# OpenMined/CampX

Measured on AMD Instinct MI355X. Metric: env-steps/sec at batch=65536, boat_race 5x5, 1/2/4/8 MI355X, higher is better.
Workload: dtype int8

## Files before the change

### campx_amd/_hip.py

```python

import ctypes
import os

from .gamespec import CampxSpec, CampxShapeSpec, CampxWideSpec

_LIB_PATH = os.environ.get('CAMPX_LIB') or os.path.join(
    os.path.dirname(os.path.abspath(__file__)), 'csrc', 'libcampx_hip.so')

EXPORTS = ('campx_spec_size', 'campx_flow_scratch_bytes', 'campx_spec_validate', 'campx_spec_compile',
           'campx_pair_table_bytes', 'campx_pair_table_build', 'campx_pair_table_pack',
           'campx_reset_launch',
           'campx_rollout_launch', 'campx_update_launch', 'campx_render_launch',
           'campx_update_render_launch', 'campx_update_render_shared', 'campx_flow_shared',
           'campx_shape_spec_size', 'campx_shape_spec_validate',
           'campx_shape_rollout_launch', 'campx_shape_tables_bytes', 'campx_shape_tables_build',
           'campx_shape_scratch_bytes',
           'campx_wide_spec_size', 'campx_wide_spec_validate', 'campx_wide_tables_bytes',
           'campx_wide_tables_build', 'campx_wide_reset_launch', 'campx_wide_rollout_launch',
           'campx_wide_rules_size', 'campx_wide_enumerate_launch',
           'campx_wide_update_launch', 'campx_wide_policy_update_launch',
           'campx_wide_policy_population_launch', 'campx_wide_population_plan',
           'campx_wide_learn_plan', 'campx_wide_learn_launch',
           'campx_wide_shared_plan', 'campx_wide_shared_scratch_bytes', 'campx_wide_shared_launch',
           'campx_wide_traces_plan', 'campx_wide_traces_launch',
# ... 389 lines not shown
  if lib.campx_spec_size() != ctypes.sizeof(CampxSpec):
    raise ImportError('CampxSpec layout mismatch between gamespec.py ({} B) and '
                      'libcampx_hip.so ({} B): rebuild the library'.format(
                          ctypes.sizeof(CampxSpec), lib.campx_spec_size()))
  return lib


lib = _load()

_OPS_PATH = os.path.join(os.path.dirname(_LIB_PATH), 'libcampx_torch.so')


def _load_ops():
  if not os.path.exists(_OPS_PATH):
    raise ImportError(
        '{} is missing: build it with `python -m campx_amd.build` (needs hipcc '
        'and torch). The fused tier has no CPU fallback.'.format(_OPS_PATH))
  import torch
  torch.ops.load_library(_OPS_PATH)
  return torch.ops.campx


ops = _load_ops()
OP_NAMES = ('reset', 'step', 'rollout', 'update', 'render', 'rollout_pipelined', 'update_render', 'shape_rollout', 'wide_rollout',
            'wide_update', 'wide_policy_update', 'wide_policy_population', 'wide_learn', 'wide_learn_shared', 'wide_learn_traces', 'wide_learn_dyna', 'wide_learn_actor', 'wide_learn_actor_shared', 'render_gather', 'wide_render_gather', 'wide_render_states',
            'wide_render_windows', 'returns', 'vtrace', 'state_sums', 'table_lookup', 'wide_sweeps',
            'wide_population_sweeps', 'wide_population_solve', 'wide_visit', 'wide_visit_population', 'onehot_to_ids', 'check_actions')


def check(code, what):
  if code != 0:
    raise CampxError('{} failed: {} (code {}, hipError {})'.format(
        what, lib.campx_strerror(code).decode(), code,
        lib.campx_last_hip_error()))



def config_get(name):
  value = ctypes.c_int64()
  check(lib.campx_config_get(name.encode(), ctypes.byref(value)), 'campx_config_get({!r})'.format(name))
  return int(value.value)


def config_set(name, value):
  check(lib.campx_config_set(name.encode(), int(value)), 'campx_config_set({!r}, {})'.format(name, value))

# ... 25 lines not shown
```

### campx_amd/build.py

```python

import concurrent.futures
import os
import shutil
import subprocess
import sys

HERE = os.path.dirname(os.path.abspath(__file__))
REPO = os.path.dirname(HERE)
CSRC = os.path.join(HERE, 'csrc')
UNITS = ('campx_api', 'k_interp', 'k_rollout_table', 'k_step', 'k_update', 'k_render',
         'k_shape', 'k_wide', 'k_policy', 'k_learn', 'k_gather', 'k_states', 'k_window', 'k_returns',
         'k_vtrace', 'k_sums', 'k_plan', 'k_visit', 'k_misc')
SRCS = [os.path.join(CSRC, u + '.hip') for u in UNITS]
HEADERS = [os.path.join(CSRC, 'campx_common.hip.h'), os.path.join(CSRC, 'wide_table.hip.h'),
           os.path.join(CSRC, 'streams.hip.h'), os.path.join(REPO, 'include', 'campx_hip.h')]
OBJ_DIR = os.path.join(REPO, 'build', 'obj')
OUT = os.path.join(CSRC, 'libcampx_hip.so')
INCLUDE = os.path.join(REPO, 'include')

HIPCC_FLAGS = ['--offload-arch=gfx950', '-O3', '-std=c++17', '-fPIC',
               '-ffp-contract=off', '-Wall', '-Wno-unused-function',
               '-Wno-pass-failed']


# ... 39 lines not shown
  if verbose:
    print(' '.join(cmd))
  subprocess.run(cmd, check=True)
  os.replace(out + '.tmp', out)
  return out


def build_hip(force=False, verbose=False):
  if not force and not needs_build():
    return OUT
  return link(compile_units(force=force, verbose=verbose), OUT, verbose)


TORCH_SRC = os.path.join(HERE, 'csrc', 'campx_torch.cpp')
TORCH_OUT = os.path.join(HERE, 'csrc', 'libcampx_torch.so')


def build_torch_ops(force=False, verbose=False):
  build_hip(force=False, verbose=verbose)
  if (not force and os.path.exists(TORCH_OUT) and os.path.getmtime(TORCH_OUT) >= max(
      os.path.getmtime(TORCH_SRC), os.path.getmtime(OUT),
      os.path.getmtime(os.path.join(INCLUDE, 'campx_hip.h')))):
    return TORCH_OUT
  import torch
  tdir = os.path.dirname(os.path.abspath(torch.__file__))
  cmd = [find_hipcc(), '-O2', '-std=c++17', '-shared', '-fPIC', '-DUSE_ROCM',
         '-Wno-unused-result',
         '-D_GLIBCXX_USE_CXX11_ABI={}'.format(int(torch._C._GLIBCXX_USE_CXX11_ABI)),
         '-I', INCLUDE, '-I', os.path.join(tdir, 'include'),
         '-I', os.path.join(tdir, 'include', 'torch', 'csrc', 'api', 'include'),
         TORCH_SRC, '-L', os.path.join(tdir, 'lib'), '-lc10', '-ltorch_cpu', '-ltorch',
         '-lc10_hip', '-ltorch_hip', '-L', os.path.join(HERE, 'csrc'), '-lcampx_hip',
         '-Wl,-rpath,$ORIGIN', '-o', TORCH_OUT + '.tmp']
  if verbose:
    print(' '.join(cmd))
  subprocess.run(cmd, check=True)
  os.replace(TORCH_OUT + '.tmp', TORCH_OUT)
  return TORCH_OUT


SAN_DIR = os.path.join(REPO, 'build', 'sanitize')
SAN_OUT = os.path.join(SAN_DIR, 'libcampx_hip_san.so')
SAN_FLAGS = ['--offload-host-only', '-O1', '-g', '-std=c++17', '-fPIC', '-ffp-contract=off',
             '-fsanitize=address,undefined', '-fno-sanitize-recover=undefined',
             '-fno-omit-frame-pointer', '-shared-libsan', '-Wno-unused-function', '-Wno-pass-failed']


def sanitizer_runtime():
  hipcc = find_hipcc()
  out = subprocess.run([hipcc, '-print-file-name=libclang_rt.asan-x86_64.so'],
                       stdout=subprocess.PIPE, text=True, check=True).stdout.strip()
  if not os.path.isabs(out) or not os.path.exists(out):
    raise RuntimeError('clang\'s libclang_rt.asan-x86_64.so not found (hipcc says {!r})'.format(out))
  return out

# ... 50 lines not shown
```

### campx_amd/csrc/campx_api.hip

```cpp

#include "campx_common.hip.h"

namespace campx_impl {

thread_local int32_t g_last_hip_error = 0;

struct KnobRow {
  const char* name;
  int64_t value, lo, hi;
  const char* what;
};
static KnobRow g_knobs[K_COUNT] = {
    {"trace_chunk_mb", 16, 0, 1 << 20, "MiB of trace per plane and update + render pair of a chunked rollout (all planes: x 2)"},
    {"trace_whole_mb", 28, 0, 1 << 20, "largest trace (MiB) a rollout may have and still run as one pair"},
    {"shape_chunk_kf", 2000, 1, 1 << 30, "thousand environment-frames per chunk of a frame-major shape rollout"},
    {"shape_split", 1, 0, 1, "frame-major shape kernels where the launch allows them"},
    {"big_wgs", -1, -1, 1 << 30, "big update workgroups from this many up (-1: one per CU)"},
    {"flow", 1, 0, 1, "one-launch rollouts (tagged trace) for table games up to 8 192 environments"},
    {"flow_max_naps", kFlowMaxNaps, 1, 1ll << 32, "naps before a one-launch rollout's render wave gives up"},
    {"flow_debug_delay", 0, 0, 1 << 24, "debug: delay in front of the update role's tagged stores"},
    {"wide_lds_max", (int64_t)kWideLdsMax, 0, (int64_t)kWideLdsMax, "largest state table (bytes) kept in LDS by wide_update_kernel"},
    {"wide_step", 1, 0, 1, "one-kernel Engine.play() for state-table games"},
};

static void knobs_from_environment() {
  const char* v = getenv("CAMPX_CONFIG");
  if (!v) return;
  std::string text(v);
  size_t at = 0;
  while (at < text.size()) {
    size_t end = text.find(',', at);
    if (end == std::string::npos) end = text.size();
    const std::string item = text.substr(at, end - at);
    const size_t eq = item.find('=');
    if (eq != std::string::npos) {
      const std::string name = item.substr(0, eq);
      bool known = false;
      for (KnobRow& row : g_knobs)
        if (name == row.name) {
          const long long x = atoll(item.c_str() + eq + 1);
          known = true;
          if (x >= row.lo && x <= row.hi) row.value = x;
          else fprintf(stderr, "campx: CAMPX_CONFIG: %s=%lld is outside %lld..%lld, ignored\n", row.name, x,
                       (long long)row.lo, (long long)row.hi);
        }
// ... 656 lines not shown
```

### campx_amd/csrc/campx_common.hip.h

```cpp
#ifndef CAMPX_COMMON_HIP_H_
#define CAMPX_COMMON_HIP_H_

#include <hip/hip_runtime.h>
#include <stddef.h>
#include <stdint.h>

#include <map>
#include <mutex>
#include <string>
#include <utility>
#include <stdio.h>
#include <stdlib.h>
#include <string.h>

#include "campx_hip.h"


namespace campx_impl {

constexpr int kWave = 64;
constexpr int kChunk = 64;

typedef uint32_t u32x4 __attribute__((ext_vector_type(4)));

// ... 344 lines not shown
  memset(&tp, 0, sizeof(tp));
  tp.rows = s.rows;
  tp.cols = s.cols;
  tp.n_dyn = s.n_dyn;
  tp.n_layers = s.n_layers;
  for (int d = 0; d < s.n_dyn; ++d) {
    tp.row0[d] = s.dyn_row0[d];
    tp.col0[d] = s.dyn_col0[d];
    tp.dyn_layer[d] = s.dyn_layer[d];
  }
  return tp;
}


extern thread_local int32_t g_last_hip_error;
int32_t hip_failed(hipError_t e);
inline int32_t launch_status() {
  const hipError_t e = hipGetLastError();
  return e == hipSuccess ? CAMPX_OK : hip_failed(e);
}
inline bool aligned_to(const void* p, uintptr_t n) { return (reinterpret_cast<uintptr_t>(p) & (n - 1)) == 0; }
enum Knob : int {
  K_TRACE_CHUNK_MB, K_TRACE_WHOLE_MB, K_SHAPE_CHUNK_KF, K_SHAPE_SPLIT, K_BIG_WGS, K_FLOW,
  K_FLOW_MAX_NAPS, K_FLOW_DEBUG_DELAY, K_WIDE_LDS_MAX, K_WIDE_STEP, K_COUNT
};
int64_t knob(Knob k);
constexpr uint32_t kFlowMaxNaps = 1u << 20;
constexpr size_t kWideLdsMax = 144 * 1024;

constexpr size_t kLdsPerWorkgroup = 160 * 1024;
template <typename Kernel>
hipError_t allow_lds(Kernel kernel, size_t dynamic_bytes) {
  if (dynamic_bytes <= 64 * 1024) return hipSuccess;
  static std::mutex lock;
  static std::map<std::pair<int, const void*>, size_t> granted;
  int dev = 0;
  (void)hipGetDevice(&dev);
  const std::pair<int, const void*> key(dev, reinterpret_cast<const void*>(kernel));
  std::lock_guard<std::mutex> guard(lock);
  const auto it = granted.find(key);
  if (it != granted.end() && it->second >= dynamic_bytes) return hipSuccess;
  const hipError_t e = hipFuncSetAttribute(key.second, hipFuncAttributeMaxDynamicSharedMemorySize,
                                           (int)dynamic_bytes);
  if (e == hipSuccess) granted[key] = dynamic_bytes;
  return e;
}

// ... 97 lines not shown
```

### campx_amd/csrc/campx_torch.cpp

```cpp

#include <ATen/core/Tensor.h>
#include <ATen/core/dispatch/Dispatcher.h>
#include <ATen/core/stack.h>
#include <ATen/ops/empty.h>
#include <c10/core/impl/LocalDispatchKeySet.h>
#include <ATen/hip/impl/HIPGuardImplMasqueradingAsCUDA.h>
#include <ATen/hip/impl/HIPStreamMasqueradingAsCUDA.h>
#include <hip/hip_runtime.h>
#include <torch/library.h>

#include <map>
#include <mutex>
#include <optional>
#include <string>
#include <unordered_map>

#include "campx_hip.h"

namespace {

using at::Tensor;
using OptTensor = std::optional<Tensor>;
using DeviceGuard = c10::hip::HIPGuardMasqueradingAsCUDA;

const OptTensor kNone;

hipStream_t current_stream() { return c10::hip::getCurrentHIPStreamMasqueradingAsCUDA().stream(); }

void check_ok(int32_t rc, const char* what) {
  TORCH_CHECK(rc == CAMPX_OK, what, " failed: ", campx_strerror(rc), " (code ", rc, ", hipError ",
              campx_last_hip_error(), ")");
}

const CampxSpec* host_spec(const Tensor& spec_host) {
  TORCH_CHECK(spec_host.device().is_cpu() && spec_host.scalar_type() == at::kByte &&
                  spec_host.is_contiguous() && spec_host.numel() == (int64_t)sizeof(CampxSpec),
              "campx: spec_host must be a contiguous CPU uint8 tensor of ", sizeof(CampxSpec),
              " bytes (the CampxSpec blob)");
// ... 261 lines not shown
                  CampxState{reinterpret_cast<int8_t*>(state.data_ptr()),
                             reinterpret_cast<uint8_t*>(done.data_ptr()), opt_ptr<float>(ret), nullptr},
                  dev,
                  B,
                  wide_planes(hs),
                  hs->n_layers,
                  hs->rows,
                  hs->cols};
}

void reset(const Tensor& spec_host, const Tensor& spec_dev, Tensor& pos, Tensor& done,
           const OptTensor& ret, const OptTensor& pair_table, Tensor& obs, const OptTensor& board) {
  const Game g = unpack_game(spec_host, spec_dev, pos, done, ret, pair_table);
  want(obs, "obs", at::kChar, g.dev, {g.B, g.L, g.H, g.W});
  if (board.has_value()) want(*board, "board", at::kChar, g.dev, {g.B, g.H, g.W});
  CampxOutputs out{};
  out.obs = reinterpret_cast<int8_t*>(obs.data_ptr());
  out.board = opt_ptr<int8_t>(board);
  const DeviceGuard guard(g.dev);
  check_ok(campx_reset_launch(g.spec_host, g.spec_dev, g.state, out, g.B, current_stream()),
           "campx_reset_launch");
}

void rollout(const Tensor& spec_host, const Tensor& spec_dev, Tensor& pos, Tensor& done,
             const OptTensor& ret, const OptTensor& pair_table, const Tensor& actions, Tensor& obs,
             const OptTensor& board, const OptTensor& reward, const OptTensor& discount,
             const OptTensor& step_done, const OptTensor& perf, const OptTensor& trace,
             const OptTensor& bad_count, const OptTensor& bad_flag, bool reset_first,
             const OptTensor& scratch, const OptTensor& scratch_state, const OptTensor& error_flag) {
  const Game g = unpack_game(spec_host, spec_dev, pos, done, ret, pair_table);
  const int64_t T = want_actions("campx::rollout", actions, g.dev, g.B);
  TORCH_CHECK(T <= 0x7fffffff, "campx::rollout: too many frames");
  CampxOutputs out{};
  want_frames(out, g.dev, Frames::kAsGiven, T, g.B, g.L, g.H, g.W, obs, board);
  int64_t pitch = 0;
  if (trace.has_value()) want_trace(*trace, at::kByte, g.dev, g.K, T, g.B, pitch);
  want_streams(out, g.dev, T, g.B, pitch, true, reward, discount, step_done, perf, bad_count, bad_flag);
  out.trace = opt_ptr<uint8_t>(trace);
  if (scratch.has_value()) {
    TORCH_CHECK(scratch->device() == g.dev && scratch->scalar_type() == at::kInt &&
                    scratch->is_contiguous() && scratch->numel() >= 4,
                "campx::rollout: scratch must be a contiguous int32 tensor on ", g.dev);
    out.overlap_ctl = reinterpret_cast<uint32_t*>(scratch->data_ptr());
    out.overlap_ctl_bytes = scratch->numel() * 4;
    if (scratch_state.has_value()) {
      TORCH_CHECK(scratch_state->device().is_cpu() && scratch_state->scalar_type() == at::kLong &&
                      scratch_state->is_contiguous() &&
                      scratch_state->numel() * 8 == (int64_t)sizeof(CampxFlowState),
                  "campx::rollout: scratch_state must be a contiguous CPU int64 tensor of ",
                  sizeof(CampxFlowState) / 8, " elements");
      out.flow_state = reinterpret_cast<CampxFlowState*>(scratch_state->data_ptr());
    }
  }
  out.error_flag = flag_ptr(error_flag, g.dev);
  const DeviceGuard guard(g.dev);
  check_ok(campx_rollout_launch(g.spec_host, g.spec_dev, g.state, ids(actions), out, g.B, (int32_t)T,
                                reset_first ? 1 : 0, current_stream()),
           "campx_rollout_launch");
}

void update(const Tensor& spec_host, const Tensor& spec_dev, Tensor& pos, Tensor& done,
            const OptTensor& ret, const OptTensor& pair_table, const Tensor& actions,
            const OptTensor& reward, const OptTensor& discount, const OptTensor& step_done,
            const OptTensor& perf, Tensor& trace, const OptTensor& bad_count,
            const OptTensor& bad_flag, bool reset_first) {
  const Game g = unpack_game(spec_host, spec_dev, pos, done, ret, pair_table);
  const int64_t T = want_actions("campx::update", actions, g.dev, g.B);
  TORCH_CHECK(T >= 1 && T <= 0x7fffffff, "campx::update: bad frame count");
  int64_t pitch = 0;
  want_trace(trace, at::kByte, g.dev, g.K, T, g.B, pitch);
  CampxOutputs out{};
  want_streams(out, g.dev, T, g.B, pitch, true, reward, discount, step_done, perf, bad_count, bad_flag);
  out.trace = reinterpret_cast<uint8_t*>(trace.data_ptr());
  const DeviceGuard guard(g.dev);
  check_ok(campx_update_launch(g.spec_host, g.spec_dev, g.state, ids(actions), out, g.B, (int32_t)T,
                               reset_first ? 1 : 0, current_stream()),
           "campx_update_launch");
}

void render(const Tensor& spec_host, const Tensor& spec_dev, const Tensor& trace, Tensor& obs,
            const OptTensor& board) {
  const CampxSpec* hs = host_spec(spec_host);
// ... 85 lines not shown
void update_render(const Tensor& spec_host, const Tensor& spec_dev, Tensor& pos, Tensor& done,
                   const OptTensor& ret, const OptTensor& pair_table, const Tensor& actions,
                   const OptTensor& reward, const OptTensor& discount, const OptTensor& step_done,
                   const OptTensor& perf, Tensor& trace, const OptTensor& bad_count,
                   const OptTensor& bad_flag, bool reset_first, const Tensor& prev_trace,
                   Tensor& prev_obs) {
  const Game g = unpack_game(spec_host, spec_dev, pos, done, ret, pair_table);
  const int64_t T = want_actions("campx::update_render", actions, g.dev, g.B);
  TORCH_CHECK(T >= 1 && T <= 65535, "campx::update_render: 1 to 65535 frames");
  int64_t pitch = 0;
  CampxOutputs out{}, prev{};
  want_trace(trace, at::kByte, g.dev, g.K, T, g.B, pitch);
  want_trace(prev_trace, at::kByte, g.dev, g.K, T, g.B, prev.scalar_pitch);
  TORCH_CHECK(prev_trace.data_ptr() != trace.data_ptr(),
              "campx::update_render: the two rollouts need a trace buffer each");
  want_streams(out, g.dev, T, g.B, pitch, true, reward, discount, step_done, perf, bad_count, bad_flag);
  out.trace = reinterpret_cast<uint8_t*>(trace.data_ptr());
  want_frames(prev, g.dev, Frames::kEvery, T, g.B, g.L, g.H, g.W, prev_obs, kNone, "prev_obs");
  prev.trace = reinterpret_cast<uint8_t*>(prev_trace.data_ptr());
  const DeviceGuard guard(g.dev);
  check_ok(campx_update_render_launch(g.spec_host, g.spec_dev, g.state, ids(actions), out, prev, g.B,
                                      (int32_t)T, reset_first ? 1 : 0, current_stream()),
           "campx_update_render_launch");
}

void step(const Tensor& spec_host, const Tensor& spec_dev, Tensor& pos, Tensor& done,
          const OptTensor& ret, const OptTensor& pair_table, const Tensor& actions, Tensor& obs,
          const OptTensor& board, const OptTensor& reward, const OptTensor& discount,
          const OptTensor& step_done, const OptTensor& perf, const OptTensor& bad_count,
          const OptTensor& bad_flag) {
  const Game g = unpack_game(spec_host, spec_dev, pos, done, ret, pair_table);
  want(actions, "actions", at::kChar, g.dev, {g.B});
  CampxOutputs out{};
  want_frames(out, g.dev, Frames::kOne, 1, g.B, g.L, g.H, g.W, obs, board);
  want_streams(out, g.dev, 1, g.B, 0, false, reward, discount, step_done, perf, bad_count, bad_flag);
  const DeviceGuard guard(g.dev);
  check_ok(campx_rollout_launch(g.spec_host, g.spec_dev, g.state, ids(actions), out, g.B, 1, 0,
                                current_stream()),
           "campx_rollout_launch");
}

void shape_rollout(const Tensor& spec_host, const Tensor& spec_dev, Tensor& pos, Tensor& done,
                   const OptTensor& ret, const OptTensor& backdrop_state, const OptTensor& actions,
                   Tensor& obs, const OptTensor& board, const OptTensor& reward,
                   const OptTensor& discount, const OptTensor& step_done,
                   const OptTensor& bad_count, const OptTensor& bad_flag, bool reset_first,
                   bool emit_first, const OptTensor& trace, const OptTensor& tables) {
  const CampxShapeSpec* hs = static_cast<const CampxShapeSpec*>(
      host_blob(spec_host, sizeof(CampxShapeSpec), "CampxShapeSpec"));
  TORCH_CHECK(pos.device().is_cuda() && pos.dim() == 2,
              "campx::shape_rollout: state must be on a HIP device (no CPU implementation)");
  const c10::Device dev = pos.device();
  const int64_t B = pos.size(1), N = hs->n_things, L = hs->n_layers, H = hs->rows, W = hs->cols;
  want(pos, "pos", at::kChar, dev, {2 * N, B});
  want(done, "done", at::kByte, dev, {B});
  if (ret.has_value()) want(*ret, "ret", at::kFloat, dev, {B});
  if (backdrop_state.has_value()) want(*backdrop_state, "backdrop_state", at::kChar, dev, {B, H * W});
  const CampxShapeSpec* ds = static_cast<const CampxShapeSpec*>(
      dev_blob(spec_dev, sizeof(CampxShapeSpec), "CampxShapeSpec", dev));
  int64_t T = 0;
  bool frames = false;
  if (actions.has_value()) {
// ... 1181 lines not shown
  m.impl("wide_render_windows", &wide_render_windows);
  m.impl("returns", &returns);
  m.impl("vtrace", &vtrace);
  m.impl("state_sums", &state_sums);
  m.impl("table_lookup", &table_lookup);
  m.impl("wide_sweeps", &wide_sweeps);
  m.impl("wide_population_sweeps", &wide_population_sweeps);
  m.impl("wide_population_solve", &wide_population_solve);
  m.impl("wide_visit", &wide_visit);
  m.impl("wide_visit_population", &wide_visit_population);
  m.impl("onehot_to_ids", &onehot_to_ids);
  m.impl("check_actions", &check_actions);
}

TORCH_LIBRARY_IMPL(campx, ADInplaceOrView, m) {
  for (const char* name : kOps)
    m.impl(name, torch::CppFunction::makeFromBoxedFunction<&run_then_bump_versions>());
}

TORCH_LIBRARY_IMPL(campx, Meta, m) {
  for (const char* name : kOps)
    m.impl(name, torch::CppFunction::makeFromBoxedFunction<&nothing_to_infer>());
}
```

### campx_amd/fused.py

```python

import ctypes
import os

import torch

from . import _hip
from . import gamespec
from .rendering import Observation


COMPILE_TABLE = True
SPLIT_ROLLOUT = True
FORCE_SPLIT = SPLIT_ROLLOUT
PAD_ROWS = True

_OBS_DTYPES = (torch.int8, torch.float16, torch.bfloat16)
GATHER_STREAMING = True


def _ptr(t):
  return ctypes.c_void_p(t.data_ptr()) if t is not None else ctypes.c_void_p(0)



# ... 76 lines not shown
        _hip.check(rc, 'campx_pair_table_build')
    self.uses_table = self.uses_table or self._pair_table is not None
    self.pos = torch.zeros((2 * self.n_dyn, B), dtype=torch.int8, device=dev)
    self.done = torch.zeros((B,), dtype=torch.uint8, device=dev)
    self.ret = torch.zeros((B,), dtype=torch.float32, device=dev)
    self._obs = torch.empty((B, self.n_layers, self.rows, self.cols),
                            dtype=torch.int8, device=dev)
    self._board = torch.empty((B, self.rows, self.cols), dtype=torch.int8,
                              device=dev)
    self._reward = torch.empty((B,), dtype=torch.float32, device=dev)
    self._discount = torch.empty((B,), dtype=torch.float32, device=dev)
    self._step_done = torch.empty((B,), dtype=torch.uint8, device=dev)
    self.perf = torch.zeros((B,), dtype=torch.int8, device=dev)
    self._perf_arg = self.perf if self.has_perf else None
    self._bad = torch.zeros((1,), dtype=torch.int32, device=dev)
    self._onehot_bad = torch.zeros((1,), dtype=torch.int32, device=dev)
    self._bad_flag = torch.zeros((1,), dtype=torch.int32).pin_memory()
    self._bad_flag_view = self._bad_flag.numpy()
    self.validate_actions = True
    self.frame = -1
    self._observation_cache = self._observation(self._obs, self._board)
    self._step = _hip.ops.step.default
    self._rollout = _hip.ops.rollout.default
    self._update = _hip.ops.update.default
    self._render = _hip.ops.render.default
    self._update_render = _hip.ops.update_render.default
    self._rollout_pipelined = _hip.ops.rollout_pipelined.default
    self._flow_scratch = None
    self._flow_state = None
    self._flow_shared = {}
    self._err_flag = torch.zeros((1,), dtype=torch.int32).pin_memory()
    self._err_flag_view = self._err_flag.numpy()
    self._init_gather()
    self._deferred = None
    self._deferred_rendered = False
    self._shared_launch = {}
    self._aux_in_sync = False


  def _observation(self, obs, board):
    layers = {ch: obs[:, i] for i, ch in enumerate(self.chars)}
    return Observation(board=board, layers=layers, layered_board=obs)

  def _init_gather(self):
    self._bad_idx = torch.zeros((1,), dtype=torch.int32, device=self.device)
    self._bad_idx_flag = torch.zeros((1,), dtype=torch.int32).pin_memory()
# ... 98 lines not shown
                   self._pair_table, self._obs, self._board)
    self.frame = 0
    return self._observation_cache, None, 1.0

  def reset(self):
    if self._obs.dtype != torch.int8:
      first = torch.empty(self._obs.shape, dtype=torch.int8, device=self.device)
      _hip.ops.reset(self._spec_host, self._spec_dev, self.pos, self.done, self.ret,
                     self._pair_table, first, self._board)
      self._obs.copy_(first)
      self.frame = 0
      return self._observation_cache, None, 1.0
    return self.showtime()

  def set_play_obs_dtype(self, dtype):
    if dtype not in _OBS_DTYPES:
      raise ValueError('obs dtype must be torch.int8, float16 or bfloat16')
    if dtype != torch.int8 and not self.uses_table:
      raise ValueError('16-bit play() observations need a game with a tabulated update pass')
    if dtype != self._obs.dtype:
      shown = self._obs.to(dtype)
      self._obs = shown
      self._observation_cache = self._observation(self._obs, self._board)

  def play(self, actions):
    if (torch.is_tensor(actions) and actions.dtype == torch.int8
        and actions.device == self.device and actions.shape == (self.batch,)
        and actions.is_contiguous()):
      ids = actions
    else:
      ids = self._action_ids(actions, (self.batch,))
    validate = self.validate_actions
    self._aux_in_sync = False
    self._step(self._spec_host, self._spec_dev, self.pos, self.done, self.ret,
               self._pair_table, ids, self._obs, self._board, self._reward,
               self._discount, self._step_done, self._perf_arg,
               self._bad if validate else None,
               self._bad_flag if validate else None)
    self.frame += 1
    if validate:
      self._after_launch()
    return (self._observation_cache,
            (self._reward if self.any_reward else None), self._discount)

  def capture_play(self, n_frames, policy=None, record_obs=False):
    from .play_graph import PlayGraph
    return PlayGraph(self, n_frames, policy=policy, record_obs=record_obs)

  def _one_launch(self, T, pitch):
    key = (T, pitch)
    got = self._flow_shared.get(key)
    if got is None:
      got = self._flow_shared[key] = bool(_hip.lib.campx_flow_shared(
          ctypes.byref(self.spec), self.batch, T, pitch))
    return got

  def _scratch(self, T, out):
    trace = out.get('trace')
    if trace is None or out['obs'].dim() != 5 or out['obs'].dtype != torch.int8:
      return None, None
    if not self._one_launch(T, trace.stride(1)):
      return None, None
    need = (int(_hip.lib.campx_flow_scratch_bytes(self.batch, T)) + 3) // 4
    if self._flow_scratch is None or self._flow_scratch.numel() < need:
      self._flow_scratch = torch.zeros(need, dtype=torch.int32, device=self.device)
      self._flow_state = torch.zeros(ctypes.sizeof(_hip.CampxFlowState) // 8, dtype=torch.int64)
    return self._flow_scratch, self._flow_state

  def rollout_buffers(self, T, keep_obs=True, want_board=False,
                      obs_dtype=torch.int8, share=None):
    B, L, H, W, dev = self.batch, self.n_layers, self.rows, self.cols, self.device
    if obs_dtype not in _OBS_DTYPES:
      raise ValueError('obs_dtype must be torch.int8, float16 or bfloat16')
    sixteen = obs_dtype != torch.int8
    if sixteen and not keep_obs:
      raise ValueError('16-bit observations need keep_obs=True')
    if not keep_obs and self._obs.dtype != torch.int8:
      raise ValueError('keep_obs=False renders into play()\'s frame buffer, which '
                       'set_play_obs_dtype() made {}: set it back to int8 first'
                       .format(self._obs.dtype))
    if share is not None:
      obs, board = share['obs'], share['board']
    else:
      obs = (torch.empty((T, B, L, H, W), dtype=obs_dtype, device=dev)
             if keep_obs else self._obs)
      board = None
      if want_board:
        board = (torch.empty((T, B, H, W), dtype=torch.int8, device=dev)
                 if keep_obs else self._board)
    split = SPLIT_ROLLOUT or sixteen
# ... 1 lines not shown

    def rows(dtype, *lead):
      return torch.empty(lead + (T, pitch), dtype=dtype, device=dev)[..., :B]
    return dict(
        obs=obs, board=board,
        reward=rows(torch.float32) if self.any_reward else None,
        discount=rows(torch.float32),
        done=rows(torch.uint8),
        perf=rows(torch.int8) if self.has_perf else None,
        trace=rows(torch.uint8, self.n_dyn) if split else None)

  def rollout(self, actions, obs=None, board=None, keep_obs=True,
              reset_first=False, want_board=False, obs_dtype=torch.int8,
              out=None, pipelined=False):
    T = int(actions.shape[0])
    if T < 1:
      raise ValueError('a rollout needs at least one frame: actions [T, B] with T >= 1')
    if (torch.is_tensor(actions) and actions.dtype == torch.int8
        and actions.device == self.device and actions.shape == (T, self.batch)
        and actions.is_contiguous()):
      ids = actions
    else:
      ids = self._action_ids(actions, (T, self.batch))
    if out is None:
      B, L, H, W, dev = self.batch, self.n_layers, self.rows, self.cols, self.device
      if obs is not None and keep_obs and (
          tuple(obs.shape) != (T, B, L, H, W) or obs.dtype != obs_dtype
          or not obs.is_contiguous() or obs.device != dev):
        raise ValueError('obs must be a contiguous {} [T,B,L,H,W] tensor on {}'
                         .format(obs_dtype, dev))
      out = self.rollout_buffers(T, keep_obs, want_board or board is not None,
                                 obs_dtype)
      if obs is not None and keep_obs:
        out['obs'] = obs
      if board is not None:
        out['board'] = board
    validate = self.validate_actions
    if pipelined:
      if out['trace'] is None:
        raise ValueError('pipelined rollouts need the two-kernel path (a trace buffer: '
                         'keep_obs=True on a game whose update pass is tabulated)')
      self._rollout_pipelined(self._spec_host, self._spec_dev, self.pos, self.done, self.ret,
                              self._pair_table, ids, out['obs'], out['board'], out['reward'],
                              out['discount'], out['done'], out['perf'], out['trace'],
                              self._bad if validate else None,
                              self._bad_flag if validate else None, bool(reset_first),
                              not self._aux_in_sync or ids is not actions or pipelined == 'resync')
      self._aux_in_sync = True
    else:
      self._aux_in_sync = False
      self._rollout(self._spec_host, self._spec_dev, self.pos, self.done, self.ret,
                    self._pair_table, ids, out['obs'], out['board'], out['reward'],
                    out['discount'], out['done'], out['perf'], out['trace'],
                    self._bad if validate else None,
                    self._bad_flag if validate else None, bool(reset_first),
                    *(self._scratch(T, out) + (self._err_flag,)))
    self.frame = T if reset_first else self.frame + T
    self.check_ok()
    if validate:
      self._after_launch()
    return out


  def _trace_only_refusal(self):
    if not self.uses_table:
      return ('the update pass of this game is not tabulated (it runs the rule interpreter: '
              'fused.COMPILE_TABLE is off, or its table would be too large)')
    return None

  def rollout_trace_buffers(self, T):
    B, dev = self.batch, self.device
    pitch = (B + 15) // 16 * 16 if PAD_ROWS else B

    def rows(dtype, *lead):
      return torch.empty(lead + (T, pitch), dtype=dtype, device=dev)[..., :B]
    return dict(
        reward=rows(torch.float32) if self.any_reward else None,
        discount=rows(torch.float32),
        done=rows(torch.uint8),
# ... 101 lines not shown
            out['reward'], out['discount'], out['done'], out['perf'], out['trace'],
            self._bad if validate else None, self._bad_flag if validate else None,
            bool(reset_first))
    if not one_launch or out['obs'].dtype != torch.int8:
      if prev is not None and prev['obs'].data_ptr() == out['obs'].data_ptr():
        if not self._deferred_rendered:
          self._render(self._spec_host, self._spec_dev, prev['trace'], prev['obs'], None)
        self._aux_in_sync = False
        self._update(*head)
        self._deferred, self._deferred_rendered = out, False
        self.frame = T if reset_first else self.frame + T
        self.check_ok()
        if validate:
          self._after_launch()
        return prev
      self.flush()
      if (actions_ready and out['obs'].dtype == torch.int8 and
          self.batch > 8192 and (self.n_dyn >= 3 or self.batch < 32768)):
        self.rollout(ids, out=out, reset_first=reset_first,
                     pipelined='resync' if ids is not actions else True)
        self._deferred, self._deferred_rendered = out, True
        return prev
      self._aux_in_sync = False
      self._rollout(self._spec_host, self._spec_dev, self.pos, self.done, self.ret,
                    self._pair_table, ids, out['obs'], None, out['reward'], out['discount'],
                    out['done'], out['perf'], out['trace'], self._bad if validate else None,
                    self._bad_flag if validate else None, bool(reset_first),
                    *(self._scratch(T, out) + (self._err_flag,)))
      self._deferred, self._deferred_rendered = out, True
      self.frame = T if reset_first else self.frame + T
      self.check_ok()
      if validate:
        self._after_launch()
      return prev
    self._aux_in_sync = False
    share = (prev is not None and not self._deferred_rendered
             and tuple(prev['trace'].shape) == tuple(out['trace'].shape))
    if prev is not None and not share:
      self.flush()
    if share:
      self._update_render(*(head + (prev['trace'], prev['obs'])))
    else:
      self._update(*head)
    self._deferred, self._deferred_rendered = out, False
    self.frame = T if reset_first else self.frame + T
    self.check_ok()
    if validate:
      self._after_launch()
    return prev

  def flush(self):
# ... 10 lines not shown
```

### campx_amd/play_graph.py

```python

import gc

import torch


class _no_collection(object):

  def __enter__(self):
    gc.collect()
    self.was_enabled = gc.isenabled()
    gc.disable()

  def __exit__(self, *exc):
    if self.was_enabled:
      gc.enable()


class PlayGraph(object):

  def __init__(self, fused, n_frames, policy=None, record_obs=False, warmup=2):
    n = int(n_frames)
    if n < 1:
      raise ValueError('capture_play() needs at least one frame')
    if fused.validate_actions == 'sync':
# ... 20 lines not shown
    side.wait_stream(torch.cuda.current_stream(dev))
    with torch.cuda.stream(side):
      for _ in range(max(1, warmup)):
        self._frames()
        for t, kept in zip(state, saved):
          t.copy_(kept)
    torch.cuda.current_stream(dev).wait_stream(side)
    torch.cuda.synchronize(dev)
    with _no_collection(), torch.cuda.graph(self._graph):
      self._frames()
    f.frame = frame0
    self._captured = (f._obs.data_ptr(), f._board.data_ptr())

  def _frames(self):
    f = self.fused
    single = (f._reward, f._discount, f._step_done, getattr(f, '_perf_arg', None))
    try:
      with torch.no_grad():
        self._frames_no_grad()
    finally:
      f._reward, f._discount, f._step_done = single[:3]
      if self.perf is not None:
        f._perf_arg = single[3]

  def _frames_no_grad(self):
    f = self.fused
    for t in range(self.n):
      if self.obs is not None:
        self.obs[t].copy_(f._obs)
      if self.policy is not None:
        ids = self.policy(f._observation_cache, t)
        if tuple(ids.shape) != (f.batch,):
          raise ValueError('the policy must return action ids of shape [B] = [{}], got {}'.format(
              f.batch, tuple(ids.shape)))
        self.actions[t].copy_(ids)
      f._reward = self.reward[t] if self.reward is not None else f._reward
      f._discount, f._step_done = self.discount[t], self.done[t]
      if self.perf is not None:
        f._perf_arg = self.perf[t]
      f.play(self.actions[t])

  @property
  def observation(self):
    return self.fused._observation_cache

  def replay(self, actions=None):
    f = self.fused
    if (f._obs.data_ptr(), f._board.data_ptr()) != self._captured:
      raise RuntimeError('the engine\'s frame buffers are not the ones this graph was captured with '
                         '(set_play_obs_dtype() after capture_play()?): capture again')
    if actions is not None:
      if self.policy is not None:
        raise ValueError('this graph was captured with a policy: it chooses the actions')
      actions = torch.as_tensor(actions)
      if tuple(actions.shape) != (self.n, f.batch):
        raise ValueError('actions must have shape {}, got {}'.format((self.n, f.batch), tuple(actions.shape)))
      if actions.dtype != torch.int8:
        actions = actions.to(f.device).clamp(-1, 5)
      self.actions.copy_(actions, non_blocking=True)
    self._graph.replay()
    f.frame += self.n
    if getattr(f, '_aux_in_sync', None) is not None:
# ... 5 lines not shown
```

### campx_amd/wide.py

```python

import ctypes
import math

import torch

from . import _hip
from . import fused
from . import gamespec
from . import tabulate


STATE_TABLE_ONLY = (
    'rollout_policy_buffers', 'rollout_policy', 'rollout_population_buffers', 'rollout_population',
    'learner_buffers', 'learn_tabular', 'shared_learner_buffers', 'learn_shared', 'learn_traces', 'dyna_buffers', 'learn_dyna', 'learn_actor_critic', 'shared_actor_buffers', 'learn_actor_critic_shared', 'table_arrays', 'sweep_buffers', 'evaluate_policy',
    'value_iteration', 'population_sweep_buffers', 'evaluate_population', 'value_iteration_population',
    'visitation_buffers',
    'state_visitation', 'visit_population_buffers', 'visit_population', 'render_states', 'render_frame_windows', 'render_trace_windows', 'render_state_windows')


def refuse_state_table_only(tier, answers=None):
  def refusal(name, answer):
    def refuse(self, *args, **kwargs):
      getattr(self, answer)(name)
    refuse.__name__ = name
# ... 77 lines not shown
    self._bad_visit_member_rows = torch.zeros((1,), dtype=torch.int32, device=dev)
    self._bad_state_ids = torch.zeros((1,), dtype=torch.int32, device=dev)
    self._states_scratch = []
    self._bad_window_rows = torch.zeros((1,), dtype=torch.int32, device=dev)
    self._bad_window_ids = torch.zeros((1,), dtype=torch.int32, device=dev)
    self._bad_learners = torch.zeros((1,), dtype=torch.int32, device=dev)
    self._bad_shared_learners = torch.zeros((1,), dtype=torch.int32, device=dev)
    self._bad_trace_learners = torch.zeros((1,), dtype=torch.int32, device=dev)
    self._bad_dyna_learners = torch.zeros((1,), dtype=torch.int32, device=dev)
    self._bad_actor_learners = torch.zeros((1,), dtype=torch.int32, device=dev)
    self._bad_actor_rows = torch.zeros((1,), dtype=torch.int32, device=dev)
    self._bad_shared_actor_learners = torch.zeros((1,), dtype=torch.int32, device=dev)
    self._bad_shared_actor_rows = torch.zeros((1,), dtype=torch.int32, device=dev)
    self._hyper_floats = {}
    self._hyper_ints = {}
    self._layer_of_cell = None
    self._window_table()
    self._bad_flag = torch.zeros((1,), dtype=torch.int32).pin_memory()
    self._bad_flag_view = self._bad_flag.numpy()
    self.validate_actions = True
    self.frame = -1
    self._observation_cache = self._observation(self._obs, self._board)
    self._wide = _hip.ops.wide_rollout.default
    self._err_flag = torch.zeros((1,), dtype=torch.int32).pin_memory()
    self._err_flag_view = self._err_flag.numpy()
    self._init_gather()
    bad_row = '(a weight that is negative or NaN, or a sum that is not a positive finite number)'
    acts, idx = self._bad_flag_view, self._bad_idx_flag_view
    self._lazy_errors.insert(1, (
        self._bad_rows, acts,
        '{} environment-frames of rollout_policy() met bad policy rows ' + bad_row + '; they took action {}'))
    self._lazy_errors.insert(2, (
        self._bad_member_rows, acts,
        '{} environment-frames of rollout_population() met bad policy rows ' + bad_row +
        '; they took action {}'))
    self._lazy_errors += [
        (self._bad_state_ids, idx,
         '{} state ids of render_states() are outside the game\'s table (they were rendered as state 0)'),
        (self._bad_plan_rows, acts,
         '{} rows of the policy given to evaluate_policy() are bad ' + bad_row +
         '; they were evaluated as taking action {}'),
        (self._bad_population_rows, acts,
         '{} rows of the policies given to evaluate_population() are bad ' + bad_row +
         '; they were evaluated as taking action {}'),
        (self._bad_visit_rows, acts,
         '{} rows of the policy given to state_visitation() are bad ' + bad_row +
# ... 1143 lines not shown
```

Measured before the change: 35.63 billion.

## Bind step and rollout launches into cached plans to skip per-call op dispatch

Adds pybind-exposed StepPlan and RolloutPlan objects that validate and unpack tensors once, then relaunch the rollout kernel directly on later calls and bump the version counters of written tensors by hand. Engine.play() and rollout() keep a small cache of plans, keyed by output buffers, frame count and validation mode, and fall back to the dispatcher op when plans are disabled or the cache misses. This targets the PyTorch dispatcher and argument-checking cost per launch, which dominates for small, fast kernels. The cost is cache-invalidation complexity: stale bindings are a risk if buffers change without _drop_plans being called.

```diff
diff --git a/campx_amd/_hip.py b/campx_amd/_hip.py
--- a/campx_amd/_hip.py
+++ b/campx_amd/_hip.py
@@ -435,6 +435,19 @@
 
 
 ops = _load_ops()
+
+
+def _load_plans():
+  import importlib.machinery
+  import importlib.util
+  loader = importlib.machinery.ExtensionFileLoader('_campx_plans', _OPS_PATH)
+  spec = importlib.util.spec_from_file_location('_campx_plans', _OPS_PATH, loader=loader)
+  module = importlib.util.module_from_spec(spec)
+  loader.exec_module(module)
+  return module
+
+
+plans = _load_plans()
 OP_NAMES = ('reset', 'step', 'rollout', 'update', 'render', 'rollout_pipelined', 'update_render', 'shape_rollout', 'wide_rollout',
             'wide_update', 'wide_policy_update', 'wide_policy_population', 'wide_learn', 'wide_learn_shared', 'wide_learn_traces', 'wide_learn_dyna', 'wide_learn_actor', 'wide_learn_actor_shared', 'render_gather', 'wide_render_gather', 'wide_render_states',
             'wide_render_windows', 'returns', 'vtrace', 'state_sums', 'table_lookup', 'wide_sweeps',
diff --git a/campx_amd/build.py b/campx_amd/build.py
--- a/campx_amd/build.py
+++ b/campx_amd/build.py
@@ -85,6 +85,7 @@
       os.path.getmtime(TORCH_SRC), os.path.getmtime(OUT),
       os.path.getmtime(os.path.join(INCLUDE, 'campx_hip.h')))):
     return TORCH_OUT
+  import sysconfig
   import torch
   tdir = os.path.dirname(os.path.abspath(torch.__file__))
   cmd = [find_hipcc(), '-O2', '-std=c++17', '-shared', '-fPIC', '-DUSE_ROCM',
@@ -92,8 +93,9 @@
          '-D_GLIBCXX_USE_CXX11_ABI={}'.format(int(torch._C._GLIBCXX_USE_CXX11_ABI)),
          '-I', INCLUDE, '-I', os.path.join(tdir, 'include'),
          '-I', os.path.join(tdir, 'include', 'torch', 'csrc', 'api', 'include'),
+         '-I', sysconfig.get_paths()['include'], '-fvisibility-inlines-hidden',
          TORCH_SRC, '-L', os.path.join(tdir, 'lib'), '-lc10', '-ltorch_cpu', '-ltorch',
-         '-lc10_hip', '-ltorch_hip', '-L', os.path.join(HERE, 'csrc'), '-lcampx_hip',
+         '-lc10_hip', '-ltorch_hip', '-ltorch_python', '-L', os.path.join(HERE, 'csrc'), '-lcampx_hip',
          '-Wl,-rpath,$ORIGIN', '-o', TORCH_OUT + '.tmp']
   if verbose:
     print(' '.join(cmd))
diff --git a/campx_amd/csrc/campx_api.hip b/campx_amd/csrc/campx_api.hip
--- a/campx_amd/csrc/campx_api.hip
+++ b/campx_amd/csrc/campx_api.hip
@@ -21,6 +21,7 @@
     {"flow_debug_delay", 0, 0, 1 << 24, "debug: delay in front of the update role's tagged stores"},
     {"wide_lds_max", (int64_t)kWideLdsMax, 0, (int64_t)kWideLdsMax, "largest state table (bytes) kept in LDS by wide_update_kernel"},
     {"wide_step", 1, 0, 1, "one-kernel Engine.play() for state-table games"},
+    {"launch_plans", 1, 0, 1, "bound launch plans behind Engine.play() / rollout() instead of an op dispatch per call"},
 };
 
 static void knobs_from_environment() {
diff --git a/campx_amd/csrc/campx_common.hip.h b/campx_amd/csrc/campx_common.hip.h
--- a/campx_amd/csrc/campx_common.hip.h
+++ b/campx_amd/csrc/campx_common.hip.h
@@ -390,7 +390,8 @@
 inline bool aligned_to(const void* p, uintptr_t n) { return (reinterpret_cast<uintptr_t>(p) & (n - 1)) == 0; }
 enum Knob : int {
   K_TRACE_CHUNK_MB, K_TRACE_WHOLE_MB, K_SHAPE_CHUNK_KF, K_SHAPE_SPLIT, K_BIG_WGS, K_FLOW,
-  K_FLOW_MAX_NAPS, K_FLOW_DEBUG_DELAY, K_WIDE_LDS_MAX, K_WIDE_STEP, K_COUNT
+  K_FLOW_MAX_NAPS, K_FLOW_DEBUG_DELAY, K_WIDE_LDS_MAX, K_WIDE_STEP, K_LAUNCH_PLANS,
+  K_COUNT
 };
 int64_t knob(Knob k);
 constexpr uint32_t kFlowMaxNaps = 1u << 20;
diff --git a/campx_amd/csrc/campx_torch.cpp b/campx_amd/csrc/campx_torch.cpp
--- a/campx_amd/csrc/campx_torch.cpp
+++ b/campx_amd/csrc/campx_torch.cpp
@@ -8,12 +8,14 @@
 #include <ATen/hip/impl/HIPStreamMasqueradingAsCUDA.h>
 #include <hip/hip_runtime.h>
 #include <torch/library.h>
+#include <torch/csrc/utils/pybind.h>
 
 #include <map>
 #include <mutex>
 #include <optional>
 #include <string>
 #include <unordered_map>
+#include <vector>
 
 #include "campx_hip.h"
 
@@ -321,16 +323,37 @@
            "campx_reset_launch");
 }
 
-void rollout(const Tensor& spec_host, const Tensor& spec_dev, Tensor& pos, Tensor& done,
-             const OptTensor& ret, const OptTensor& pair_table, const Tensor& actions, Tensor& obs,
-             const OptTensor& board, const OptTensor& reward, const OptTensor& discount,
-             const OptTensor& step_done, const OptTensor& perf, const OptTensor& trace,
-             const OptTensor& bad_count, const OptTensor& bad_flag, bool reset_first,
-             const OptTensor& scratch, const OptTensor& scratch_state, const OptTensor& error_flag) {
-  const Game g = unpack_game(spec_host, spec_dev, pos, done, ret, pair_table);
-  const int64_t T = want_actions("campx::rollout", actions, g.dev, g.B);
-  TORCH_CHECK(T <= 0x7fffffff, "campx::rollout: too many frames");
-  CampxOutputs out{};
+struct Bound {
+  Game g;
+  CampxOutputs out;
+  int64_t T;
+  bool frames;
+};
+
+Bound bind_step(const Tensor& spec_host, const Tensor& spec_dev, const Tensor& pos, const Tensor& done,
+                const OptTensor& ret, const OptTensor& pair_table, const Tensor& actions,
+                const Tensor& obs, const OptTensor& board, const OptTensor& reward,
+                const OptTensor& discount, const OptTensor& step_done, const OptTensor& perf,
+                const OptTensor& bad_count, const OptTensor& bad_flag) {
+  Bound b{unpack_game(spec_host, spec_dev, pos, done, ret, pair_table), CampxOutputs{}, 1, false};
+  want(actions, "actions", at::kChar, b.g.dev, {b.g.B});
+  want_frames(b.out, b.g.dev, Frames::kOne, 1, b.g.B, b.g.L, b.g.H, b.g.W, obs, board);
+  want_streams(b.out, b.g.dev, 1, b.g.B, 0, false, reward, discount, step_done, perf, bad_count, bad_flag);
+  return b;
+}
+
+Bound bind_rollout(const char* what, const Tensor& spec_host, const Tensor& spec_dev, const Tensor& pos,
+                   const Tensor& done, const OptTensor& ret, const OptTensor& pair_table,
+                   const Tensor& actions, const Tensor& obs, const OptTensor& board,
+                   const OptTensor& reward, const OptTensor& discount, const OptTensor& step_done,
+                   const OptTensor& perf, const OptTensor& trace, const OptTensor& bad_count,
+                   const OptTensor& bad_flag, const OptTensor& scratch, const OptTensor& scratch_state,
+                   const OptTensor& error_flag) {
+  Bound b{unpack_game(spec_host, spec_dev, pos, done, ret, pair_table), CampxOutputs{}, 0, true};
+  const Game& g = b.g;
+  CampxOutputs& out = b.out;
+  const int64_t T = b.T = want_actions(what, actions, g.dev, g.B);
+  TORCH_CHECK(T <= 0x7fffffff, what, ": too many frames");
   want_frames(out, g.dev, Frames::kAsGiven, T, g.B, g.L, g.H, g.W, obs, board);
   int64_t pitch = 0;
   if (trace.has_value()) want_trace(*trace, at::kByte, g.dev, g.K, T, g.B, pitch);
@@ -339,24 +362,159 @@
   if (scratch.has_value()) {
     TORCH_CHECK(scratch->device() == g.dev && scratch->scalar_type() == at::kInt &&
                     scratch->is_contiguous() && scratch->numel() >= 4,
-                "campx::rollout: scratch must be a contiguous int32 tensor on ", g.dev);
+                what, ": scratch must be a contiguous int32 tensor on ", g.dev);
     out.overlap_ctl = reinterpret_cast<uint32_t*>(scratch->data_ptr());
     out.overlap_ctl_bytes = scratch->numel() * 4;
     if (scratch_state.has_value()) {
       TORCH_CHECK(scratch_state->device().is_cpu() && scratch_state->scalar_type() == at::kLong &&
                       scratch_state->is_contiguous() &&
                       scratch_state->numel() * 8 == (int64_t)sizeof(CampxFlowState),
-                  "campx::rollout: scratch_state must be a contiguous CPU int64 tensor of ",
+                  what, ": scratch_state must be a contiguous CPU int64 tensor of ",
                   sizeof(CampxFlowState) / 8, " elements");
       out.flow_state = reinterpret_cast<CampxFlowState*>(scratch_state->data_ptr());
     }
   }
   out.error_flag = flag_ptr(error_flag, g.dev);
-  const DeviceGuard guard(g.dev);
-  check_ok(campx_rollout_launch(g.spec_host, g.spec_dev, g.state, ids(actions), out, g.B, (int32_t)T,
-                                reset_first ? 1 : 0, current_stream()),
+  return b;
+}
+
+void want_ids(const Bound& b, const Tensor& actions) {
+  if (b.frames) want(actions, "actions", at::kChar, b.g.dev, {b.T, b.g.B});
+  else want(actions, "actions", at::kChar, b.g.dev, {b.g.B});
+}
+
+void launch(const Bound& b, const Tensor& actions, bool reset_first) {
+  const DeviceGuard guard(b.g.dev);
+  check_ok(campx_rollout_launch(b.g.spec_host, b.g.spec_dev, b.g.state, ids(actions), b.out, b.g.B,
+                                (int32_t)b.T, reset_first ? 1 : 0, current_stream()),
            "campx_rollout_launch");
 }
+
+void rollout(const Tensor& spec_host, const Tensor& spec_dev, Tensor& pos, Tensor& done,
+             const OptTensor& ret, const OptTensor& pair_table, const Tensor& actions, Tensor& obs,
+             const OptTensor& board, const OptTensor& reward, const OptTensor& discount,
+             const OptTensor& step_done, const OptTensor& perf, const OptTensor& trace,
+             const OptTensor& bad_count, const OptTensor& bad_flag, bool reset_first,
+             const OptTensor& scratch, const OptTensor& scratch_state, const OptTensor& error_flag) {
+  launch(bind_rollout("campx::rollout", spec_host, spec_dev, pos, done, ret, pair_table, actions, obs,
+                      board, reward, discount, step_done, perf, trace, bad_count, bad_flag, scratch,
+                      scratch_state, error_flag),
+         actions, reset_first);
+}
+
+void step(const Tensor& spec_host, const Tensor& spec_dev, Tensor& pos, Tensor& done,
+          const OptTensor& ret, const OptTensor& pair_table, const Tensor& actions, Tensor& obs,
+          const OptTensor& board, const OptTensor& reward, const OptTensor& discount,
+          const OptTensor& step_done, const OptTensor& perf, const OptTensor& bad_count,
+          const OptTensor& bad_flag) {
+  launch(bind_step(spec_host, spec_dev, pos, done, ret, pair_table, actions, obs, board, reward,
+                   discount, step_done, perf, bad_count, bad_flag),
+         actions, false);
+}
+
+const Tensor* arg(const Tensor& t) { return &t; }
+const Tensor* arg(const OptTensor& t) { return t.has_value() ? &*t : nullptr; }
+
+std::vector<Tensor> written_by(const char* op, std::initializer_list<const Tensor*> args) {
+  const auto& arguments = c10::Dispatcher::singleton().findSchemaOrThrow(op, "").schema().arguments();
+  TORCH_INTERNAL_ASSERT(arguments.size() == args.size(), op, ": the plan and the schema disagree");
+  std::vector<Tensor> written;
+  size_t i = 0;
+  for (const Tensor* t : args) {
+    const c10::AliasInfo* alias = arguments[i++].alias_info();
+    if (t && t->defined() && alias && alias->isWrite()) written.push_back(*t);
+  }
+  return written;
+}
+
+bool plans_enabled() {
+  int64_t on = 1;
+  (void)campx_config_get("launch_plans", &on);
+  return on != 0;
+}
+
+class LaunchPlan {
+ public:
+  LaunchPlan(const Bound& bound, std::vector<Tensor> keep, const std::vector<Tensor>& written,
+             const OptTensor& ret)
+      : bound_(bound), keep_(std::move(keep)), ret_(ret.has_value() ? *ret : Tensor()) {
+    for (const Tensor& t : written)
+      if (!t.is_same(ret_) && !t.is_inference()) written_.push_back(t.unsafeGetTensorImpl());
+  }
+
+  bool run(const Tensor& actions, bool reset_first, const OptTensor& ret) {
+    if (!plans_enabled()) return false;
+    want_ids(bound_, actions);
+    at::TensorImpl* given = ret.has_value() ? ret->unsafeGetTensorImpl() : nullptr;
+    if (given != (ret_.defined() ? ret_.unsafeGetTensorImpl() : nullptr)) {
+      if (given) want(*ret, "ret", at::kFloat, bound_.g.dev, {bound_.g.B});
+      bound_.g.state.ret = opt_ptr<float>(ret);
+      ret_ = given ? *ret : Tensor();
+    }
+    launch(bound_, actions, reset_first);
+    for (at::TensorImpl* t : written_) t->bump_version();
+    if (given && !ret_.is_inference()) given->bump_version();
+    return true;
+  }
+
+ private:
+  Bound bound_;
+  std::vector<Tensor> keep_;
+  std::vector<at::TensorImpl*> written_;
+  Tensor ret_;
+};
+
+std::vector<Tensor> present(std::initializer_list<const Tensor*> args) {
+  std::vector<Tensor> keep;
+  for (const Tensor* t : args)
+    if (t && t->defined()) keep.push_back(*t);
+  return keep;
+}
+
+struct StepPlan : LaunchPlan {
+  StepPlan(const Tensor& spec_host, const Tensor& spec_dev, const Tensor& pos, const Tensor& done,
+           const OptTensor& ret, const OptTensor& pair_table, const Tensor& actions, const Tensor& obs,
+           const OptTensor& board, const OptTensor& reward, const OptTensor& discount,
+           const OptTensor& step_done, const OptTensor& perf, const OptTensor& bad_count,
+           const OptTensor& bad_flag)
+      : LaunchPlan(bind_step(spec_host, spec_dev, pos, done, ret, pair_table, actions, obs, board, reward,
+                             discount, step_done, perf, bad_count, bad_flag),
+                   present({arg(spec_host), arg(spec_dev), arg(pos), arg(done), arg(pair_table), arg(obs),
+                            arg(board), arg(reward), arg(discount), arg(step_done), arg(perf),
+                            arg(bad_count), arg(bad_flag)}),
+                   written_by("campx::step",
+                              {arg(spec_host), arg(spec_dev), arg(pos), arg(done), arg(ret),
+                               arg(pair_table), arg(actions), arg(obs), arg(board), arg(reward),
+                               arg(discount), arg(step_done), arg(perf), arg(bad_count), arg(bad_flag)}),
+                   ret) {}
+  bool step(const Tensor& actions, const OptTensor& ret) { return run(actions, false, ret); }
+};
+
+struct RolloutPlan : LaunchPlan {
+  RolloutPlan(const Tensor& spec_host, const Tensor& spec_dev, const Tensor& pos, const Tensor& done,
+              const OptTensor& ret, const OptTensor& pair_table, const Tensor& actions, const Tensor& obs,
+              const OptTensor& board, const OptTensor& reward, const OptTensor& discount,
+              const OptTensor& step_done, const OptTensor& perf, const OptTensor& trace,
+              const OptTensor& bad_count, const OptTensor& bad_flag, const OptTensor& scratch,
+              const OptTensor& scratch_state, const OptTensor& error_flag)
+      : LaunchPlan(bind_rollout("campx::rollout", spec_host, spec_dev, pos, done, ret, pair_table, actions,
+                                obs, board, reward, discount, step_done, perf, trace, bad_count, bad_flag,
+                                scratch, scratch_state, error_flag),
+                   present({arg(spec_host), arg(spec_dev), arg(pos), arg(done), arg(pair_table), arg(obs),
+                            arg(board), arg(reward), arg(discount), arg(step_done), arg(perf), arg(trace),
+                            arg(bad_count), arg(bad_flag), arg(scratch), arg(scratch_state),
+                            arg(error_flag)}),
+                   written_by("campx::rollout",
+                              {arg(spec_host), arg(spec_dev), arg(pos), arg(done), arg(ret),
+                               arg(pair_table), arg(actions), arg(obs), arg(board), arg(reward),
+                               arg(discount), arg(step_done), arg(perf), arg(trace), arg(bad_count),
+                               arg(bad_flag), nullptr , arg(scratch),
+                               arg(scratch_state), arg(error_flag)}),
+                   ret) {}
+  bool rollout(const Tensor& actions, bool reset_first, const OptTensor& ret) {
+    return run(actions, reset_first, ret);
+  }
+};
 
 void update(const Tensor& spec_host, const Tensor& spec_dev, Tensor& pos, Tensor& done,
             const OptTensor& ret, const OptTensor& pair_table, const Tensor& actions,
@@ -488,22 +646,6 @@
   check_ok(campx_update_render_launch(g.spec_host, g.spec_dev, g.state, ids(actions), out, prev, g.B,
                                       (int32_t)T, reset_first ? 1 : 0, current_stream()),
            "campx_update_render_launch");
-}
-
-void step(const Tensor& spec_host, const Tensor& spec_dev, Tensor& pos, Tensor& done,
-          const OptTensor& ret, const OptTensor& pair_table, const Tensor& actions, Tensor& obs,
-          const OptTensor& board, const OptTensor& reward, const OptTensor& discount,
-          const OptTensor& step_done, const OptTensor& perf, const OptTensor& bad_count,
-          const OptTensor& bad_flag) {
-  const Game g = unpack_game(spec_host, spec_dev, pos, done, ret, pair_table);
-  want(actions, "actions", at::kChar, g.dev, {g.B});
-  CampxOutputs out{};
-  want_frames(out, g.dev, Frames::kOne, 1, g.B, g.L, g.H, g.W, obs, board);
-  want_streams(out, g.dev, 1, g.B, 0, false, reward, discount, step_done, perf, bad_count, bad_flag);
-  const DeviceGuard guard(g.dev);
-  check_ok(campx_rollout_launch(g.spec_host, g.spec_dev, g.state, ids(actions), out, g.B, 1, 0,
-                                current_stream()),
-           "campx_rollout_launch");
 }
 
 void shape_rollout(const Tensor& spec_host, const Tensor& spec_dev, Tensor& pos, Tensor& done,
@@ -1731,3 +1873,27 @@
   for (const char* name : kOps)
     m.impl(name, torch::CppFunction::makeFromBoxedFunction<&nothing_to_infer>());
 }
+
+PYBIND11_MODULE(_campx_plans, m) {
+  namespace py = pybind11;
+  py::register_local_exception_translator([](std::exception_ptr p) {
+    try {
+      if (p) std::rethrow_exception(p);
+    } catch (const c10::Error& e) {
+      PyErr_SetString(PyExc_RuntimeError, e.what_without_backtrace());
+    }
+  });
+  py::class_<StepPlan>(m, "StepPlan")
+      .def(py::init<const Tensor&, const Tensor&, const Tensor&, const Tensor&, const OptTensor&,
+                    const OptTensor&, const Tensor&, const Tensor&, const OptTensor&, const OptTensor&,
+                    const OptTensor&, const OptTensor&, const OptTensor&, const OptTensor&,
+                    const OptTensor&>())
+      .def("step", &StepPlan::step, py::arg("actions"), py::arg("ret"));
+  py::class_<RolloutPlan>(m, "RolloutPlan")
+      .def(py::init<const Tensor&, const Tensor&, const Tensor&, const Tensor&, const OptTensor&,
+                    const OptTensor&, const Tensor&, const Tensor&, const OptTensor&, const OptTensor&,
+                    const OptTensor&, const OptTensor&, const OptTensor&, const OptTensor&,
+                    const OptTensor&, const OptTensor&, const OptTensor&, const OptTensor&,
+                    const OptTensor&>())
+      .def("rollout", &RolloutPlan::rollout, py::arg("actions"), py::arg("reset_first"), py::arg("ret"));
+}
diff --git a/campx_amd/fused.py b/campx_amd/fused.py
--- a/campx_amd/fused.py
+++ b/campx_amd/fused.py
@@ -122,6 +122,8 @@
     self._observation_cache = self._observation(self._obs, self._board)
     self._step = _hip.ops.step.default
     self._rollout = _hip.ops.rollout.default
+    self._step_plans = {}
+    self._rollout_plans = {}
     self._update = _hip.ops.update.default
     self._render = _hip.ops.render.default
     self._update_render = _hip.ops.update_render.default
@@ -266,6 +268,17 @@
       shown = self._obs.to(dtype)
       self._obs = shown
       self._observation_cache = self._observation(self._obs, self._board)
+      self._drop_plans()
+
+  def _drop_plans(self):
+    self._step_plans.clear()
+
+  def _step_plan(self, validate, ids):
+    plan = self._step_plans[validate] = _hip.plans.StepPlan(
+        self._spec_host, self._spec_dev, self.pos, self.done, self.ret, self._pair_table, ids,
+        self._obs, self._board, self._reward, self._discount, self._step_done, self._perf_arg,
+        self._bad if validate else None, self._bad_flag if validate else None)
+    return plan
 
   def play(self, actions):
     if (torch.is_tensor(actions) and actions.dtype == torch.int8
@@ -276,11 +289,13 @@
       ids = self._action_ids(actions, (self.batch,))
     validate = self.validate_actions
     self._aux_in_sync = False
-    self._step(self._spec_host, self._spec_dev, self.pos, self.done, self.ret,
-               self._pair_table, ids, self._obs, self._board, self._reward,
-               self._discount, self._step_done, self._perf_arg,
-               self._bad if validate else None,
-               self._bad_flag if validate else None)
+    plan = self._step_plans.get(validate) or self._step_plan(validate, ids)
+    if not plan.step(ids, self.ret):
+      self._step(self._spec_host, self._spec_dev, self.pos, self.done, self.ret,
+                 self._pair_table, ids, self._obs, self._board, self._reward,
+                 self._discount, self._step_done, self._perf_arg,
+                 self._bad if validate else None,
+                 self._bad_flag if validate else None)
     self.frame += 1
     if validate:
       self._after_launch()
@@ -310,6 +325,43 @@
       self._flow_scratch = torch.zeros(need, dtype=torch.int32, device=self.device)
       self._flow_state = torch.zeros(ctypes.sizeof(_hip.CampxFlowState) // 8, dtype=torch.int64)
     return self._flow_scratch, self._flow_state
+
+  _PLAN_KEYS = ('obs', 'board', 'reward', 'discount', 'done', 'perf', 'trace')
+  _PLANS_KEPT = 4
+
+  def _launch_rollout(self, ids, out, T, validate, reset_first, planned):
+    if planned:
+      validated = bool(validate)
+      entry = self._rollout_plans.get(id(out))
+      fits = entry is not None and entry[1] == T and entry[2] == validated
+      if fits:
+        for key, bound in zip(self._PLAN_KEYS, entry[3]):
+          if out.get(key) is not bound:
+            fits = False
+            break
+      if fits and entry[4] is not None and entry[4] is not self._flow_scratch:
+        fits = False
+      if fits:
+        plan = entry[0]
+      else:
+        scratch, scratch_state = self._scratch(T, out)
+        tensors = tuple(out.get(key) for key in self._PLAN_KEYS)
+        plan = _hip.plans.RolloutPlan(
+            self._spec_host, self._spec_dev, self.pos, self.done, self.ret, self._pair_table, ids,
+            *(tensors + (self._bad if validate else None, self._bad_flag if validate else None,
+                         scratch, scratch_state, self._err_flag)))
+        self._rollout_plans.pop(id(out), None)
+        while len(self._rollout_plans) >= self._PLANS_KEPT:
+          del self._rollout_plans[next(iter(self._rollout_plans))]
+        self._rollout_plans[id(out)] = (plan, T, validated, tensors, scratch)
+      if plan.rollout(ids, bool(reset_first), self.ret):
+        return
+    self._rollout(self._spec_host, self._spec_dev, self.pos, self.done, self.ret,
+                  self._pair_table, ids, out['obs'], out['board'], out['reward'],
+                  out['discount'], out['done'], out['perf'], out['trace'],
+                  self._bad if validate else None,
+                  self._bad_flag if validate else None, bool(reset_first),
+                  *(self._scratch(T, out) + (self._err_flag,)))
 
   def rollout_buffers(self, T, keep_obs=True, want_board=False,
                       obs_dtype=torch.int8, share=None):
@@ -357,6 +409,7 @@
       ids = actions
     else:
       ids = self._action_ids(actions, (T, self.batch))
+    planned = out is not None
     if out is None:
       B, L, H, W, dev = self.batch, self.n_layers, self.rows, self.cols, self.device
       if obs is not None and keep_obs and (
@@ -384,12 +437,7 @@
       self._aux_in_sync = True
     else:
       self._aux_in_sync = False
-      self._rollout(self._spec_host, self._spec_dev, self.pos, self.done, self.ret,
-                    self._pair_table, ids, out['obs'], out['board'], out['reward'],
-                    out['discount'], out['done'], out['perf'], out['trace'],
-                    self._bad if validate else None,
-                    self._bad_flag if validate else None, bool(reset_first),
-                    *(self._scratch(T, out) + (self._err_flag,)))
+      self._launch_rollout(ids, out, T, validate, reset_first, planned)
     self.frame = T if reset_first else self.frame + T
     self.check_ok()
     if validate:
@@ -537,11 +585,7 @@
         self._deferred, self._deferred_rendered = out, True
         return prev
       self._aux_in_sync = False
-      self._rollout(self._spec_host, self._spec_dev, self.pos, self.done, self.ret,
-                    self._pair_table, ids, out['obs'], None, out['reward'], out['discount'],
-                    out['done'], out['perf'], out['trace'], self._bad if validate else None,
-                    self._bad_flag if validate else None, bool(reset_first),
-                    *(self._scratch(T, out) + (self._err_flag,)))
+      self._launch_rollout(ids, out, T, validate, reset_first, True)
       self._deferred, self._deferred_rendered = out, True
       self.frame = T if reset_first else self.frame + T
       self.check_ok()
diff --git a/campx_amd/play_graph.py b/campx_amd/play_graph.py
--- a/campx_amd/play_graph.py
+++ b/campx_amd/play_graph.py
@@ -66,6 +66,12 @@
       f._reward, f._discount, f._step_done = single[:3]
       if self.perf is not None:
         f._perf_arg = single[3]
+      self._rebound()
+
+  def _rebound(self):
+    drop = getattr(self.fused, '_drop_plans', None)
+    if drop is not None:
+      drop()
 
   def _frames_no_grad(self):
     f = self.fused
@@ -82,6 +88,7 @@
       f._discount, f._step_done = self.discount[t], self.done[t]
       if self.perf is not None:
         f._perf_arg = self.perf[t]
+      self._rebound()
       f.play(self.actions[t])
 
   @property
diff --git a/campx_amd/wide.py b/campx_amd/wide.py
--- a/campx_amd/wide.py
+++ b/campx_amd/wide.py
@@ -123,6 +123,7 @@
     self.frame = -1
     self._observation_cache = self._observation(self._obs, self._board)
     self._wide = _hip.ops.wide_rollout.default
+    self._step_plans = {}
     self._err_flag = torch.zeros((1,), dtype=torch.int32).pin_memory()
     self._err_flag_view = self._err_flag.numpy()
     self._init_gather()
```

Result: no change. 35.59 billion (-0.1%).
